# NREL/sup3r

Measured on AMD Instinct MI355X. Metric: samples/sec (lo-res chunks), generator forward, 5x/12x ST-GAN, higher is better.
Workload: dtype bf16

## Files before the change

### include/sup3r_hip.h

```cpp
#ifndef SUP3R_HIP_H
#define SUP3R_HIP_H

#include <stdint.h>

#ifdef __cplusplus
extern "C" {
#endif

#define S3_OK 0
#define S3_EINVAL (-1)
#define S3_EHIP (-2)
#define S3_ENOMEM (-3)
#define S3_ERCCL (-4)
#define S3_ESTATE (-5)
#define S3_ETIMEOUT (-6)

enum {
  S3_OP_CONV = 1,
  S3_OP_REPEAT_T = 2,
  S3_OP_D2S = 3,
  S3_OP_ACT = 4,
  S3_OP_ADD = 5,
  S3_OP_CONCAT = 6,
  S3_OP_DENSE = 7,
  S3_OP_PAD = 8,
  S3_OP_CROP = 9,
  S3_OP_VIEW = 10,
  S3_OP_ROLL_T = 11,
  S3_OP_DILATE = 12
};
enum { S3_ACT_NONE = 0, S3_ACT_RELU = 1, S3_ACT_LEAKY = 2 };
enum { S3_PAD_ZERO = 0, S3_PAD_REFLECT = 1 };
enum {
  S3_PREC_F32 = 0,
  S3_PREC_BF16 = 1,
  S3_PREC_BF16X3 = 2
};
enum { S3_LOSS_MAE = 0, S3_LOSS_MSE = 1, S3_LOSS_EXP = 2 };
enum { S3_BUF_W = 0, S3_BUF_G = 1, S3_BUF_M = 2, S3_BUF_V = 3 };

typedef struct s3_ctx s3_ctx;
typedef struct s3_params s3_params;
typedef struct s3_plan s3_plan;

typedef struct {
  int64_t dims[5];
} s3_tensor_desc;

typedef struct {
  int32_t kind;
  int32_t in0, in1, res, out;
  int32_t w, b;
  int32_t k[3], stride[3], lo[3], hi[3];
  int32_t pad_mode;
  int32_t act;
  float alpha;
  int32_t d2s;
  int32_t rep;
  int32_t bcast_c;
  int32_t reserved[4];
} s3_op_desc;

int s3_ctx_create(int device_id, void* stream, int create_stream, s3_ctx** out);
void s3_ctx_destroy(s3_ctx* ctx);
const char* s3_last_error(const s3_ctx* ctx);
int s3_ctx_sync(s3_ctx* ctx);
void* s3_ctx_stream(s3_ctx* ctx);
enum { S3_STAT_PERSIST_DGRAD = 0,
       S3_STAT_GCONV_SPLITK = 1,
       S3_STAT_BUCKET_ELEMS = 2,
       S3_STAT_DGRAD_C2_SLIDE = 3,
       S3_STAT_BUCKETS = 4,
       S3_STAT_ALLREDUCES = 5,
       S3_STAT_BIAS_STAGE1 = 6,
       S3_STAT_BIAS_STAGE1_V4 = 7,
       S3_STAT_BIAS_COLS = 8,
       S3_STAT_BIAS_COLS_SPLIT = 9,
       S3_STAT_BIAS_PARTIAL = 10,
       S3_STAT_BIAS_PARTIAL_RIDE = 11,
       S3_STAT_BIAS_PARTIAL_FLUSH = 12,
       S3_STAT_EPI_GENERIC = 13,
       S3_STAT_EPI_C4 = 14,
       S3_STAT_EPI_D2S4 = 15,
       S3_STAT_EPI_C4_BSUM = 16,
       S3_STAT_EPI_D2S4_BSUM = 17,
       S3_STAT_FOLD_GATHER = 18,
       S3_STAT_FOLD_PAD4 = 19,
       S3_STAT_FOLD_PAD4_FR16 = 20,
       S3_STAT_FOLD16X8 = 21,
       S3_STAT_FOLD_PLAIN = 22,
       S3_STAT_FOLD_MASKED = 23,
       S3_STAT_FOLD_ADD = 24,
       S3_STAT_AXPY = 25,
       S3_STAT_AXPY4 = 26,
       S3_STAT_PERSIST_SKIPPRE = 27,
       S3_STAT_HALO_S2_K64 = 28,
       S3_STAT_FEWCH_HALO = 29,
       S3_STAT_FEWCH_HALO_SIGNS = 30,
       S3_STAT_DGRAD_S2_O16 = 31,
       S3_STAT_DGRAD_S2_MB = 32,
       S3_STAT_COUNT = 33 };
int64_t s3_ctx_stat(const s3_ctx* ctx, int which);

int s3_params_create(s3_ctx* ctx, int n, const int64_t* sizes, s3_params** out);
void s3_params_destroy(s3_params* p);
int64_t s3_params_total(const s3_params* p);
int s3_params_set(s3_params* p, int which, int idx, const float* host);
int s3_params_get(s3_params* p, int which, int idx, float* host);
void* s3_params_dptr(s3_params* p, int which, int idx);
int s3_params_zero_grad(s3_params* p);
uint64_t s3_params_version(const s3_params* p);
int s3_params_mean_abs(s3_params* p, int which, int idx, float* host_out);

int s3_adam_step(s3_params* p, float lr, float beta1, float beta2, float eps,
                 int64_t t);
typedef enum {
  S3_OPT_ADAM = 0, S3_OPT_SGD = 1, S3_OPT_RMSPROP = 2, S3_OPT_ADAGRAD = 3,
  S3_OPT_ADAMAX = 4, S3_OPT_ADAMW = 5
} s3_optimizer_kind;
int s3_optimizer_step(s3_params* p, int kind, const double* hp, int n_hp,
                      int64_t t);
int s3_optimizer_stage(s3_params* p, int kind, const double* hp, int n_hp,
                       int64_t t);
int s3_optimizer_step_staged(s3_params* p, int kind);
int s3_params_touch(s3_params* p);

typedef struct s3_graph s3_graph;
int s3_capture_begin(s3_ctx* ctx);
int s3_capture_end(s3_ctx* ctx, s3_graph** out);
int s3_capture_abort(s3_ctx* ctx);
int s3_graph_launch(s3_graph* g);
int64_t s3_graph_nodes(const s3_graph* g);
void s3_graph_destroy(s3_graph* g);

#define S3_OPTION_UNSET INT32_MIN
typedef struct {
  int32_t n;
  const char* const* names;
  const int32_t* values;
} s3_plan_options;
int s3_ctx_set_option(s3_ctx* ctx, const char* name, int32_t value);
int s3_ctx_get_option(const s3_ctx* ctx, const char* name, int32_t* value);
const char* s3_option_name_at(int index);

int s3_plan_create(s3_ctx* ctx, s3_params* params, const s3_tensor_desc* tensors,
                   int n_tensors, const s3_op_desc* ops, int n_ops,
                   const int32_t* inputs, int n_inputs, int32_t output,
                   int precision, int training, s3_plan** out);
int s3_plan_create_opt(s3_ctx* ctx, s3_params* params, const s3_tensor_desc* tensors,
                       int n_tensors, const s3_op_desc* ops, int n_ops,
                       const int32_t* inputs, int n_inputs, int32_t output,
                       int precision, int training, const s3_plan_options* options,
                       s3_plan** out);
void s3_plan_destroy(s3_plan* plan);
int s3_plan_forward(s3_plan* plan, const void* const* inputs, void* output);
int s3_plan_supports_window(const s3_plan* plan);
int s3_plan_forward_window(s3_plan* plan, const void* const* inputs, void* output,
                           const int64_t* lo3, const int64_t* n3,
                           const float* affine_dev, int n_c);
int s3_plan_backward(s3_plan* plan, const void* d_output, void* d_input,
                     int need_wgrad, int accumulate_wgrad);
void* s3_plan_tensor(s3_plan* plan, int32_t tensor_id);
int64_t s3_plan_workspace_bytes(const s3_plan* plan);
int s3_plan_profile_begin(s3_plan* plan, int max_forwards);
int s3_plan_profile_end(s3_plan* plan, float* ms_per_op, int cap);
int s3_plan_op_is_mfma(const s3_plan* plan, int op_index);
enum {
  S3_OPINFO_KIND = 0,
  S3_OPINFO_FWD = 1,
  S3_OPINFO_IN16 = 2,
  S3_OPINFO_OUT16 = 3,
  S3_OPINFO_RES16 = 4,
  S3_OPINFO_FWD_BF16_OPS = 5,
  S3_OPINFO_WGRAD = 6,
  S3_OPINFO_DGRAD = 7,
  S3_OPINFO_MASK_FUSED_FROM = 8,
  S3_OPINFO_IN_REP = 9,
  S3_OPINFO_RES_REP = 10,
  S3_OPINFO_DGRAD_FRAME16 = 11,
  S3_OPINFO_FEWPOS_MFMA = 12,
  S3_OPINFO_COUNT = 13
};
enum {
  S3_FWD_DIRECT = 0, S3_FWD_MFMA_TILE = 1, S3_FWD_MFMA_PERSIST = 2, S3_FWD_GCONV = 3,
// ... 378 lines not shown
```

### sup3r_amd/_lib.py

```python
import ctypes as C
import os

HERE = os.path.dirname(os.path.abspath(__file__))
LIB_PATH = os.environ.get('SUP3R_AMD_LIB') or os.path.join(
    HERE, 'lib', 'libsup3r_hip.so')

PREC_F32, PREC_BF16, PREC_BF16X3 = 0, 1, 2
LOSS_MAE, LOSS_MSE, LOSS_EXP = 0, 1, 2
BUF_W, BUF_G, BUF_M, BUF_V = 0, 1, 2, 3
OPT_ADAM = 0
SURF_OTHER, SURF_TEMP, SURF_PRES, SURF_RH = 0, 1, 2, 3
E_TIMEOUT = -6
PRECISIONS = {'f32': PREC_F32, 'bf16': PREC_BF16, 'bf16x3': PREC_BF16X3}

EXPORTS = [
    's3_ctx_create', 's3_ctx_destroy', 's3_last_error', 's3_ctx_sync',
    's3_ctx_stream', 's3_ctx_stat', 's3_params_create', 's3_params_destroy',
    's3_params_total', 's3_params_set', 's3_params_get', 's3_params_dptr',
    's3_params_zero_grad', 's3_params_version', 's3_params_mean_abs',
    's3_adam_step', 's3_optimizer_step', 's3_optimizer_stage',
    's3_optimizer_step_staged', 's3_params_touch', 's3_capture_begin',
    's3_capture_end', 's3_capture_abort', 's3_graph_launch', 's3_graph_nodes',
    's3_graph_destroy',
    's3_ctx_set_option', 's3_ctx_get_option', 's3_option_name_at',
# ... 230 lines not shown
        's3_scale_to_time_max': (i32, [vp, vp, vp, i64, i64, vp]),
        's3_host_register': (i32, [vp, vp, C.c_size_t]),
        's3_host_unregister': (i32, [vp, vp]),
        's3_d2h_window': (i32, [vp, vp, vp, i64, i64, i64, i64, i64, vp]),
        's3_d2h_stream': (i32, [vp, vp, vp, C.c_size_t, vp, i32]),
        's3_host_alloc': (i32, [vp, C.c_size_t, i32, C.POINTER(vp)]),
        's3_host_free': (i32, [vp, vp]),
        's3_d2h_async': (i32, [vp, vp, vp, C.c_size_t, vp]),
        's3_dma_d2h_begin': (i32, [vp, vp, vp, C.c_size_t,
                                   C.POINTER(C.c_uint64)]),
        's3_dma_wait': (i32, [vp, C.c_uint64, i32]),
        's3_coarsen': (i32, [vp, vp, i32, i32, i32, i32, i32, i32, i32, i32,
                             vp]),
        's3_gaussian_smooth': (i32, [vp, vp, i32, i32, i32, i32, i32, pf, i32,
                                     C.c_uint32, vp, vp]),
        's3_condmom_target': (i32, [vp, vp, vp, vp, i32, i32, i32, i32, i32,
                                    i32, i32, C.POINTER(i32), i32, i32,
                                    C.c_uint32, i32, i32, i32, vp, vp]),
        's3_sample_gather': (i32, [vp, vp, i64, i64, i64, i32, C.POINTER(i32),
                                   i32, i32, i32, i32, C.POINTER(i32), i32,
                                   vp]),
        's3_cc_night_mask': (i32, [vp, vp, i64, i64, i64, i32, C.POINTER(i32),
                                   i32, i32, i32, i32, vp]),
        's3_cc_window_gather': (i32, [vp, vp, i64, i64, i64, i32,
                                      C.POINTER(i32), i32, i32, i32, i32,
                                      C.POINTER(i32), i32, vp, vp]),
        's3_nn_fill': (i32, [vp, vp, i32, i32, i32, i32, i32, i32, vp, vp]),
        's3_channel_moments': (i32, [vp, vp, i64, i32, vp]),
        's3_normalize_channels': (i32, [vp, vp, i64, i32, pf, pf,
                                        C.POINTER(C.c_ubyte)]),
        's3_bias_correct': (i32, [vp, vp, i32, i32, i32, i32, i32,
                                  C.POINTER(BiasChannel), i32, i32,
                                  C.POINTER(i32), vp, vp, vp,
                                  C.POINTER(C.c_double),
                                  C.POINTER(C.c_double), i32, vp, vp]),
        's3_bc_base_series': (i32, [vp, vp, vp, i64, i64, i32, vp, vp, vp, vp,
                                    i32, vp, vp, vp, vp, i32, C.c_uint32, i32,
                                    i64, i64, vp]),
        's3_bc_moments': (i32, [vp, vp, i32, i64, vp, vp, i32, vp, vp, vp]),
        's3_bc_window_quantiles': (i32, [vp, vp, i32, i64, i32, vp, vp, vp,
                                         vp, i32, vp]),
        's3_bc_match_zero_rate': (i32, [vp, vp, i64, vp, i32, i64, vp, vp]),
        's3_bc_presrat': (i32, [vp, vp, i64, vp, i64, vp, i64, i32, i32, i32,
                                vp, vp, vp, i32, C.c_double, vp, vp,
                                C.POINTER(vp), C.POINTER(vp), C.POINTER(vp),
                                C.POINTER(vp), vp, vp, vp, vp, vp, vp, vp]),
        's3_st_interp': (i32, [vp, vp, i32, i32, i32, i32, i32, i32, i32, vp,
                               vp]),
        's3_resize2d': (i32, [vp, vp, i32, i32, i32, i32, i32, vp, vp, vp, vp,
                              i32, vp, vp]),
        's3_surface_downscale': (i32, [vp, vp, i32, i32, i32, i32, i32, vp, vp,
                                       vp, vp, i32, vp, vp, vp, i32, vp, u64,
                                       C.c_uint32, vp, vp, vp, vp, vp, vp]),
        's3_comm_unique_id': (i32, [vp]),
        's3_comm_init': (i32, [vp, i32, i32, vp]),
        's3_params_allreduce_grads': (i32, [vp]),
        's3_params_arm_allreduce': (i32, [vp, i64]),
        's3_allreduce_sum': (i32, [vp, vp, i64]),
        's3_comm_info': (i32, [vp, C.POINTER(i32), C.POINTER(i32)]),
        's3_params_broadcast': (i32, [vp, i32, i32]),
        's3_broadcast': (i32, [vp, vp, i64, i32]),
        's3_comm_destroy': (None, [vp]),
        's3_comm_wait': (i32, [vp, i64]),
        's3_version': (C.c_char_p, []),
    }
    for name in EXPORTS:
        fn = getattr(L, name)
        fn.restype, fn.argtypes = sig[name]
    _lib = L
    return L


STATS = {'persist_dgrad': 0, 'gconv_splitk': 1, 'bucket_elems': 2,
         'dgrad_c2_slide': 3, 'buckets': 4, 'allreduces': 5,
         'bias_stage1': 6, 'bias_stage1_v4': 7, 'bias_cols': 8,
         'bias_cols_split': 9, 'bias_partial': 10, 'bias_partial_ride': 11,
         'bias_partial_flush': 12, 'epi_generic': 13, 'epi_c4': 14,
         'epi_d2s4': 15, 'epi_c4_bsum': 16, 'epi_d2s4_bsum': 17,
         'fold_gather': 18, 'fold_pad4': 19, 'fold_pad4_fr16': 20,
         'fold16x8': 21, 'fold_plain': 22, 'fold_masked': 23, 'fold_add': 24,
         'axpy': 25, 'axpy4': 26,
         'persist_skippre': 27,
         'halo_s2_k64': 28, 'fewch_halo': 29, 'fewch_halo_signs': 30,
         'dgrad_s2_o16': 31, 'dgrad_s2_mb': 32}


def option_names():
    L, out, i = lib(), [], 0
    while True:
        name = L.s3_option_name_at(i)
        if not name:
            return out
        out.append(name.decode())
        i += 1


def plan_options(options):
    items = sorted((options or {}).items())
    n = len(items)
    names = (C.c_char_p * max(n, 1))(*[k.encode() for k, _ in items])
    values = (C.c_int32 * max(n, 1))(*[
        OPTION_UNSET if v is None else int(v) for _, v in items])
    return PlanOptions(n, names, values), (names, values)

OPINFO_FIELDS = ('kind', 'fwd', 'in16', 'out16', 'res16', 'fwd_bf16_ops',
                 'wgrad', 'dgrad', 'mask_fused_from', 'in_rep', 'res_rep',
                 'dgrad_frame16', 'fewpos_mfma')
FWD_KERNELS = ('direct', 'mfma_tile', 'mfma_persist', 'gconv', 'gconv_fewch',
               'halo32', 'fewpos', 'tail_mfma', 'small', 'fused2d', 'halo_s2',
               'mfma_gen', 'conv2d_ws', 'conv2d_head')
WGRAD_KERNELS = ('direct', 'f32_trunk', 'bf16_trunk', 'f32_gen', 'bf16_gen',
                 'bf16_2d', 'c2', 'tail', 'fewpos')
DGRAD_KERNELS = ('direct', 'mfma_frame', 'mfma_valid', 'mfma_chunked',
                 'fewch_frame', 's2', 'c2', 'gconv', 'fewpos')

TC_METHODS = {'subsample': 0, 'average': 1, 'total': 2, 'max': 3, 'min': 4}
CM_SUBFILTER, CM_LINEAR, CM_MOM1, CM_SQUARE = 1, 2, 4, 8
SAMPLE_MAX_ORIGINS, SAMPLE_MAX_CHANNELS = 64, 32
STATS_MAX_CHANNELS = 64
CC_STATUS_WORDS = 4
CC_NIGHT_MASK, CC_START_RAW, CC_START, CC_FILLED = 0, 1, 2, 3
NN_FILL_MAX_AXIS = 2048
BC_MAX_CHANNELS, BC_MAX_CHUNKS = 16, 32
BC_NONE, BC_LINEAR, BC_QDM = 0, 1, 2
(BC_MONTH, BC_WEIGHTS, BC_SCALAR_RANGE, BC_ADDER_RANGE, BC_OUT_RANGE,
 BC_PER_CHUNK, BC_RELATIVE, BC_NO_TREND, BC_DENOM_ZERO, BC_DENOM_MIN,
 BC_DELTA_RANGE, BC_PRESRAT, BC_GLOBAL) = (1 << i for i in range(13))
BCC_MAX_SORT, BCC_MAX_GROUPS = 32768, 12
BCC_AVG, BCC_MAX, BCC_MIN, BCC_SUM, BCC_NONE = range(5)
BCC_NANSKIP, BCC_CS_RATIO, BCC_ROUND = 1, 2, 4
BCC_PR_BIAS_NONFINITE, BCC_PR_FUT_NONFINITE, BCC_PR_INDEX = 0, 1, 2
LI_MAX_LEVELS, LI_MAX_SINGLE, LI_MAX_VARS, LI_MAX_TARGETS = 64, 8, 8, 16
LI_LINEAR, LI_LOG = 0, 1
LI_LEV_COLUMN, LI_LEV_VECTOR = 0, 1
(DP_UV_FROM_WSWD, DP_WSWD_FROM_UV, DP_SURFACE_RH, DP_RATIO_MASKED,
 DP_CLOUD_MASK, DP_RATIO_CLIP01, DP_ADD, DP_SCALE, DP_OFFSET, DP_BCAST_PIXEL,
 DP_BCAST_TIME) = range(11)
TF_LE, TF_NAN = 0, 1
STACK_MAX_PLANES = 32
LS_WORDS = 8
(LS_NAN, LS_BAD_MIN, LS_BAD_MAX, LS_ALL_NAN, LS_FIRST_MAX, LS_FIRST_MIN,
 LS_LAST_MAX, LS_LAST_MIN) = range(8)
EXO_MAX_SLAB = 32
QA_CUBE, QA_TIME_FIRST = 0, 1
QA_MAX_FEATURES, QA_SUMMARY_WORDS, QA_MAX_BINS = 16, 5, 4096
QA_HIST_STATS, QA_HIST_COUNTS, QA_HIST_KEEP_ALL = 1, 2, 4
RG_GRID, RG_FLAT, RG_FLAT_1D = 0, 1, 2
DAILY_MAX_SRC, DAILY_MAX_OUT = 8, 16
DAILY_MEAN, DAILY_MAX, DAILY_MIN, DAILY_SUM, DAILY_RATIO = range(5)


def last_error(ctx):
    raw = lib().s3_last_error(ctx) if ctx else None
    return raw.decode() if raw else ''


def check(rc, ctx=None, what=''):
    if rc == 0:
        return
    msg = ''
    if ctx:
        raw = lib().s3_last_error(ctx)
        msg = raw.decode() if raw else ''
    if rc == E_TIMEOUT:
        raise TimeoutError(f'sup3r_amd: {msg or what}')
    raise RuntimeError(f'sup3r_amd HIP call failed ({what}, code {rc}): {msg}')
```

### sup3r_amd/csrc/common.h

```cpp
#pragma once
#include <hip/hip_runtime.h>
#include <stdint.h>

#include <atomic>
#include <mutex>
#include <string>
#include <vector>

#include "../../include/sup3r_hip.h"
#include "launch_shape.h"


#define S3_OPTION_LIST(X) \
  X(BF16_TRAIN_ACT) \
  X(DENSE_WGS) \
  X(DGRAD_S2_MIN_TILES) \
  X(DISC_BF16) \
  X(FEWCH_HALO_MIN_TILES) \
  X(FP32_ACT) \
  X(GCONV_MF2) \
  X(GCONV_MF4) \
  X(GRAPH) \
  X(HALO32_MIN_TILES) \
  X(HALO_S2_MIN_TILES) \
  X(MFMA_DBG) \
  X(MFMA_TILE) \
  X(NO_BATCHED_PACK) \
  X(NO_BIAS_FUSE) \
  X(NO_CHUNKED_DY16) \
  X(NO_DGRAD_C2) \
  X(NO_DGRAD_C2_SLIDE) \
  X(DGRAD_C2_SLIDE_MIN_UNITS) \
  X(NO_DGRAD_CHUNKED) \
  X(NO_DGRAD_FEWCH) \
  X(NO_DGRAD_S2) \
  X(NO_DGRAD_X3) \
  X(NO_DIRECT_OUTPUT) \
  X(NO_DISC_BF16) \
  X(NO_DPRE16) \
  X(NO_DPRE16_ONLY_MASK) \
  X(NO_FEWCH) \
  X(NO_FEWCH_HALO) \
  X(NO_FEWPOS) \
  X(NO_FEWPOS_MFMA) \
  X(NO_FEWPOS_BWD_FUSE) \
  X(NO_FEWPOS_SMALL) \
  X(NO_FEWPOS_TRUNK) \
  X(NO_FOLD16) \
  X(NO_FRAME16) \
  X(NO_FUSED2D) \
  X(NO_GCONV) \
  X(NO_GCONV_DY16) \
  X(NO_GCONV_SPLITK) \
  X(NO_HALO32) \
  X(NO_HALO_S2) \
  X(NO_MASK_FUSE) \
  X(NO_MFMA_GEN) \
  X(NO_DGRAD_GEN) \
  X(NO_CONV2D_WS) \
  X(NO_TRAIN2D_BF16) \
  X(NO_ADD16) \
  X(NO_WS_EXO) \
  X(NO_WS_RES2) \
  X(NO_WS_PP) \
  X(NO_WS_X3) \
  X(WS_X3_MIN_POS) \
  X(NO_CONV2D_OUT) \
  X(NO_CONV2D_HEAD) \
  X(KEEP_ACTIVATIONS) \
  X(NO_MFMA_BWD) \
  X(NO_PERSIST) \
  X(NO_PERSIST_DGRAD) \
  X(NO_PERSIST_SKIPPRE) \
  X(NO_PERSIST_STRIP) \
  X(PERSIST2) \
  X(NO_REPEAT_FUSE) \
  X(NO_WGRAD_X3) \
  X(NO_GCONV_X3) \
  X(NO_SIGN_BYTES) \
  X(NO_HALO_S2_K64) \
  X(NO_PLAIN_FOLD16) \
  X(NO_SEG_REDUCE) \
  X(NO_TAIL_BAND) \
  X(NO_TAIL_MFMA) \
  X(NO_TAIL_SLIDE) \
  X(NO_TAIL_SWEEP) \
  X(NO_TAIL_WINDOW) \
  X(NO_TAIL_X3) \
  X(NO_TILE66) \
  X(NO_TILE_NF2) \
  X(NO_WGRAD_BF16) \
  X(NO_WGRAD_C2) \
  X(NO_WGRAD_GEN_PF) \
  X(NO_WGRAD_TAIL) \
  X(NO_WGRAD_TAIL_SWEEP) \
  X(NO_WGRAD_WS) \
  X(PERSIST_DGRAD_MIN_TILES) \
  X(PERSIST_MIN_TILES) \
  X(POISON_ALLOC) \
  X(TAIL_SWEEP_SHAPE) \
  X(TRACE) \
  X(WGRAD_DBG) \
  X(WGRAD_SIDE_STREAM)
enum S3OptId {
#define X(n) S3O_##n,
  S3_OPTION_LIST(X)
#undef X
  S3O_COUNT
};
struct S3Options {
  int32_t v[S3O_COUNT];
  bool has[S3O_COUNT];
  S3Options() { for (int i = 0; i < S3O_COUNT; ++i) { v[i] = 0; has[i] = false; } }
};
extern thread_local const S3Options* s3_active_options;
const char* s3_option_name(int id);
int s3_option_id(const char* name);
inline bool s3_opt_has(int id) { return s3_active_options && s3_active_options->has[id]; }
inline long long s3_opt_int(int id, long long dflt) { return s3_opt_has(id) ? s3_active_options->v[id] : dflt; }
inline bool s3_opt_on(int id) { return s3_opt_int(id, 0) != 0; }
struct S3OptScope {
  const S3Options* prev;
  explicit S3OptScope(const S3Options* o) : prev(s3_active_options) { s3_active_options = o; }
  ~S3OptScope() { s3_active_options = prev; }
};

struct s3_ctx {
  int device = 0;
  hipStream_t stream = nullptr;
  bool own_stream = false;
  std::string err;
  void* comm = nullptr;
  int rank = 0, nranks = 1;
  float* scratch = nullptr;
  size_t scratch_bytes = 0;
  int num_cu = 256;
  size_t lds_max = 64 * 1024;
  int64_t stat[S3_STAT_COUNT] = {};
  S3Options opt;
  hipStream_t comm_stream = nullptr;
  hipEvent_t comm_ev[2] = {nullptr, nullptr};
  hipEvent_t wd_ev[2] = {nullptr, nullptr};
  int64_t comm_issued = 0;
  hipStream_t wg_stream = nullptr;
  hipEvent_t wg_ev[2] = {nullptr, nullptr};
  bool wg_forked = false;
  hipStream_t cap_stream = nullptr, saved_stream = nullptr;
  bool capturing = false;
  bool graphs_made = false;
  std::vector<void*> retired;
  struct PendingBias { const float* partial = nullptr; int nblk = 0, c = 0; float* db = nullptr; int accumulate = 0; } pend_bias;
};

struct S3DeviceOnce {
  std::atomic<uint64_t> mask{0};
// ... 404 lines not shown
```

### sup3r_amd/csrc/kernels_conv_mfma_persist.hip

```cpp
#include <cstdlib>

#include "wave_prims.h"

namespace {

constexpr int TS0 = 4, TS1 = 8, TS2 = 16;
constexpr int H0 = TS0 + 2, H1 = TS1 + 2, H2 = TS2 + 2;
constexpr int HP = H0 * H1 * H2;
constexpr int HALO_BYTES = HP * 128;
constexpr int SLAB_OFF = HALO_BYTES;
constexpr int BIAS_OFF = SLAB_OFF + 3 * 8192;
constexpr int LDS_BYTES = BIAS_OFF + 256;

constexpr int NCW = 8;
constexpr int NPW = 4;
constexpr int NTHR = (NCW + NPW) * 64;
constexpr int MFW = TS0 * TS1 / NCW;
constexpr int PT = NPW * 64;
constexpr int ROWC = H1 * H2;
constexpr int JR = (ROWC * 8 + PT - 1) / PT;
constexpr int NLATE = (H0 - 2) * JR;
static_assert(MFW * NCW == TS0 * TS1 && TS1 % MFW == 0 && MFW == 4, "tile / wave split");
static_assert(JR <= 6 && NLATE <= 24, "producer tap schedule");

// ... 437 lines not shown
#pragma unroll
        for (int h = 0; h < 2; ++h) {
          if (2 * h >= NFV) continue;
          f32x4 a0 = acc[m][(2 * h) % NFV], a1 = acc[m][(2 * h + 1) % NFV];
          if constexpr (F16) {
            uint4 o;
            o.x = pk2(a0[0], a0[1]); o.y = pk2(a0[2], a0[3]);
            o.z = pk2(a1[0], a1[1]); o.w = pk2(a1[2], a1[3]);
            *reinterpret_cast<uint4*>(y + yo + h * 32) = o;
            continue;
          }
          if (res) {
            const float4 p0 = *reinterpret_cast<const float4*>(yp + h * 32);
            const float4 p1 = *reinterpret_cast<const float4*>(yp + h * 32 + 4);
            a0[0] += p0.x; a0[1] += p0.y; a0[2] += p0.z; a0[3] += p0.w;
            a1[0] += p1.x; a1[1] += p1.y; a1[2] += p1.z; a1[3] += p1.w;
          }
          *reinterpret_cast<float4*>(yp + h * 32) = make_float4(a0[0], a0[1], a0[2], a0[3]);
          *reinterpret_cast<float4*>(yp + h * 32 + 4) = make_float4(a1[0], a1[1], a1[2], a1[3]);
        }
      }
      WG_BARRIER();
      continue;
    }
    const size_t e_base = (size_t)n * g.O[0] * g.O[1] * g.O[2] * g.Cout;
    if constexpr (!SKP) {
      EPI_POS()
    }
#undef EPI_POS
    auto chunk_off = [&](int m, int h, bool& ok) __attribute__((always_inline)) {
      ok = c_ok[h] && e_ok[m] && 2 * h < NFV;
      return e_pos[m] + c_off[h];
    };
    if (!SKP && res) {
      const bool rr = REP > 1 && !DG && g.res_rep > 1;
      const int O2s = rr ? g.O[2] / (REP > 1 ? REP : 1) : g.O[2];
      const size_t r_base = rr ? (size_t)n * g.O[0] * g.O[1] * O2s * g.Cout : e_base;
#pragma unroll
      for (int m = 0; m < MFW; ++m) {
        unsigned r_pos = e_pos[m];
        if (rr) {
          const int mf = mf0 + m;
          const int o0 = org0 + mf / TS1, o1 = org1 + mf % TS1, o2 = org2 + frow;
          r_pos = (unsigned)(((o0 * g.O[1] + o1) * O2s + o2 / (REP > 1 ? REP : 1)) * cpo);
        }
#pragma unroll
        for (int h = 0; h < 2; ++h) {
          bool ok;
          chunk_off(m, h, ok);
          rres[m][h] = make_uint4(0, 0, 0, 0);
          if (ok) rres[m][h] = *reinterpret_cast<const uint4*>(res + r_base + r_pos + c_off[h]);
        }
      }
    }
#pragma unroll
    for (int m = 0; m < MFW; ++m) {
#pragma unroll
      for (int h = 0; h < 2; ++h) {
        bool ok;
        const unsigned off = chunk_off(m, h, ok);
        if (!ok) continue;
        float v[8];
#pragma unroll
        for (int q = 0; q < 8; ++q) {
          const float a = acc[m][(2 * h + (q >> 2)) % NFV][q & 3];
          const float sa = slope * a;
          asm("v_max_f32 %0, %1, %2" : "=v"(v[q]) : "v"(a), "v"(sa));
        }
        if (SKP || res) {
          const uint4 r = rres[m][h];
          v[0] += bf_lo(r.x); v[1] += bf_hi(r.x); v[2] += bf_lo(r.y); v[3] += bf_hi(r.y);
          v[4] += bf_lo(r.z); v[5] += bf_hi(r.z); v[6] += bf_lo(r.w); v[7] += bf_hi(r.w);
        }
        uint4 o;
        o.x = pk2(v[0], v[1]); o.y = pk2(v[2], v[3]);
        o.z = pk2(v[4], v[5]); o.w = pk2(v[6], v[7]);
        *reinterpret_cast<uint4*>(y + e_base + off) = o;
      }
    }
    WG_BARRIER();
  }
}

}

bool conv_mfma_persist_geom_ok(const ConvGeom& g) {
  if (g.Cin != 64 || g.Cout % 8 != 0 || g.Cout < 64 || g.d2s < 1) return false;
  if (g.D[2] < 8) return false;
  if (g.d2s > 1 && (g.Cout % (g.d2s * g.d2s) != 0 || (g.Cout / (g.d2s * g.d2s)) % 8 != 0))
    return false;
  if (g.pad_mode != S3_PAD_REFLECT) return false;
  if (g.act == S3_ACT_LEAKY && !(g.alpha >= 0.f && g.alpha <= 1.f)) return false;
  for (int d = 0; d < 3; ++d)
    if (g.k[d] != 3 || g.s[d] != 1) return false;
  return (int64_t)g.D[0] * g.D[1] * g.D[2] * 64 < (int64_t)1 << 31 &&
         (int64_t)g.O[0] * g.O[1] * g.O[2] * g.Cout < (int64_t)1 << 31;
}

bool conv_mfma_persist_dgrad_geom_ok(const ConvGeom& g) {
  if (g.Cin != 64 || (g.Cout != 64 && g.Cout != 32) || g.d2s != 1 || g.pad_mode != S3_PAD_ZERO ||
      g.act != S3_ACT_NONE)
    return false;
  for (int d = 0; d < 3; ++d)
    if (g.k[d] != 3 || g.s[d] != 1 || g.lo[d] != 2 || g.O[d] != g.D[d] + 2) return false;
  if (g.D[2] < 8) return false;
  if (g.in_cstride && ((g.in_cstride & 7) || (g.in_cvalid & 7) || g.in_cvalid < 8 || g.in_cvalid > 64)) return false;
  return (int64_t)g.N * g.D[0] * g.D[1] * g.D[2] * (g.in_cstride ? g.in_cstride : 64) < (int64_t)1 << 28;
}

static void persist_dgrad_grid(const ConvGeom& g, int* gs0, int* gs1) {
  int64_t best = -1;
  for (int a = 1; a <= g.N; ++a) {
    if (g.N % a) continue;
    const int b = g.N / a;
    const int64_t t = (int64_t)((a * g.O[0] + 1) / 2) * ((b * g.O[1] + TS1 - 1) / TS1);
    if (best < 0 || t < best) { best = t; *gs0 = a; *gs1 = b; }
  }
}

bool conv_mfma_persist_dgrad_supported(const s3_ctx* ctx, const ConvGeom& g) {
  if (s3_opt_on(S3O_NO_PERSIST_DGRAD)) return false;
  if (!conv_mfma_persist_dgrad_geom_ok(g)) return false;
  int gs0 = 1, gs1 = 1;
  persist_dgrad_grid(g, &gs0, &gs1);
  const int64_t halves = (int64_t)((gs0 * g.O[0] + 1) / 2) * ((gs1 * g.O[1] + TS1 - 1) / TS1) *
                         ((g.O[2] + TS2 - 1) / TS2);
  const int64_t tiles = (int64_t)((gs0 * g.O[0] + TS0 - 1) / TS0) * ((gs1 * g.O[1] + TS1 - 1) / TS1) *
                        ((g.O[2] + TS2 - 1) / TS2);
  const int64_t covered = halves * 2 * TS1 * TS2;
  const int64_t six = (int64_t)g.N * ((g.O[0] + 5) / 6) * ((g.O[1] + 5) / 6) * ((g.O[2] + 15) / 16) * 576;
  const int64_t min_tiles = s3_opt_has(S3O_PERSIST_DGRAD_MIN_TILES)
                                ? s3_opt_int(S3O_PERSIST_DGRAD_MIN_TILES, 0) : ctx->num_cu;
  return tiles >= min_tiles && covered * 10 <= six * 11;
}

int launch_conv_mfma_persist_dgrad(s3_ctx* ctx, const ConvGeom& g, const void* dpre16, const void* image,
                                   float* dxp, int accumulate, int frame16) {
  static S3DeviceOnce attr_set;
  if (int rc = s3_lds_optin(ctx, attr_set,
                            conv3_mfma_persist_kernel<4, true>, LDS_BYTES,
                            conv3_mfma_persist_kernel<2, true>, LDS_BYTES,
                            conv3_mfma_persist_kernel<4, true, 0, false, true>, LDS_BYTES)) return rc;
  if (frame16 && (accumulate || g.Cout != 64))
    S3_FAIL(ctx, S3_ESTATE, "persistent data gradient: a bf16 frame is written once, 64 channels wide");
  int gs0 = 1, gs1 = 1;
  persist_dgrad_grid(g, &gs0, &gs1);
  const int tiles0 = (gs0 * g.O[0] + 1) / 2, tiles1 = (gs1 * g.O[1] + TS1 - 1) / TS1,
            tiles2 = (g.O[2] + TS2 - 1) / TS2;
  const int n_tiles = tiles0 * tiles1 * tiles2;
  const int grid = persistent_grid(ctx->num_cu, (n_tiles + 1) / 2);
  auto kern = g.Cout <= 32 ? conv3_mfma_persist_kernel<2, true> : conv3_mfma_persist_kernel<4, true>;
  if (frame16) kern = conv3_mfma_persist_kernel<4, true, 0, false, true>;
  hipLaunchKernelGGL(kern, dim3(grid), dim3(NTHR), LDS_BYTES, ctx->stream,
                     (const unsigned short*)dpre16, (const char*)image, (const float*)nullptr,
                     (const unsigned short*)(accumulate ? dxp : nullptr), (unsigned short*)dxp, g, tiles0, tiles1,
                     tiles2, n_tiles, 0, gs0, gs1);
  S3_HIP(ctx, hipGetLastError());
  ++ctx->stat[S3_STAT_PERSIST_DGRAD];
  return S3_OK;
}

bool conv_mfma_persist_rep_ok(int rep) { return rep == 2 || rep == 3 || rep == 4; }

bool conv_mfma_persist_supported(const s3_ctx* ctx, const ConvGeom& g, ConvIO io,
                                 bool has_res) {
  if (s3_opt_on(S3O_NO_PERSIST)) return false;
  if (!io.in_bf16 || !io.out_bf16 || (has_res && !io.res_bf16)) return false;
  if (!conv_mfma_persist_geom_ok(g)) return false;
  if (has_res && g.d2s != 1) return false;
  const int64_t tiles = (int64_t)g.N * ((g.O[0] + TS0 - 1) / TS0) *
                        ((g.O[1] + TS1 - 1) / TS1) * ((g.O[2] + TS2 - 1) / TS2);
  return tiles >= s3_opt_int(S3O_PERSIST_MIN_TILES, ctx->num_cu * 7 / 16);
}

int launch_pack_jobs(s3_ctx* ctx, const S3PackJob* jobs_dev, int n_jobs, int max_ct) {
  if (n_jobs <= 0) return S3_OK;
  hipLaunchKernelGGL(pack_jobs_kernel, dim3(108 * max_ct, n_jobs), dim3(256), 0, ctx->stream, jobs_dev);
  S3_HIP(ctx, hipGetLastError());
  return S3_OK;
}

size_t conv_mfma_persist_image_bytes(const ConvGeom& g) {
  return (size_t)((g.Cout + 63) / 64) * 27 * 64 * 64 * 2;
}

int launch_conv_mfma_persist_pack(s3_ctx* ctx, const ConvGeom& g, const float* w, void* image) {
  const int n_ct = (g.Cout + 63) / 64;
  hipLaunchKernelGGL(pack_persist_kernel, dim3(108 * n_ct), dim3(256), 0, ctx->stream,
                     w, (unsigned short*)image, g.Cout, n_ct);
  S3_HIP(ctx, hipGetLastError());
  return S3_OK;
}

int launch_conv_mfma_persist(s3_ctx* ctx, const ConvGeom& g, const void* x,
                             const void* image, const float* bias,
                             const void* res, void* y) {
  static S3DeviceOnce attr_set;
#define S3_REP_ATTR(R)                                                                \
  conv3_mfma_persist_kernel<4, false, R, true>, LDS_BYTES,                            \
  conv3_mfma_persist_kernel<4, false, R, false>, LDS_BYTES,                           \
  conv3_mfma_persist_kernel<4, false, R, true, false, 6>, PGeo<6>::LDS_BYTES,         \
  conv3_mfma_persist_kernel<4, false, R, false, false, 6>, PGeo<6>::LDS_BYTES
  if (int rc = s3_lds_optin(ctx, attr_set,
                            conv3_mfma_persist_kernel<4, false>, LDS_BYTES,
                            conv3_mfma_persist_kernel<2, false>, LDS_BYTES,
                            conv3_mfma_persist_kernel<4, false, 0, false, false, 8, true>, LDS_BYTES,
                            S3_REP_ATTR(2), S3_REP_ATTR(3), S3_REP_ATTR(4),
                            conv3_mfma_persist_kernel<4, false, 0, false, false, 6>, PGeo<6>::LDS_BYTES,
                            conv3_mfma_persist_kernel<2, false, 0, false, false, 6>, PGeo<6>::LDS_BYTES)) return rc;
#undef S3_REP_ATTR
  const int tiles0 = (g.O[0] + 1) / 2, tiles1 = (g.O[1] + TS1 - 1) / TS1,
            tiles2 = (g.O[2] + TS2 - 1) / TS2;
  const int n_tiles = g.N * tiles0 * tiles1 * tiles2;
  const int grid = persistent_grid(ctx->num_cu, (n_tiles + 1) / 2);
  const int n_ct = (g.Cout + 63) / 64;
  const int rep = g.in_rep > 1 ? g.in_rep : (g.res_rep > 1 ? g.res_rep : 0);
  const bool rin = g.in_rep > 1;
  const bool skp = res && !rep && g.d2s == 1 && g.Cout == 64 && !s3_opt_on(S3O_NO_PERSIST_SKIPPRE);
  if (skp) ++ctx->stat[S3_STAT_PERSIST_SKIPPRE];
  ConvGeom gk = g;
  if (rep) {
    bool ok = conv_mfma_persist_rep_ok(rep) && g.Cout == 64 && g.d2s == 1 &&
              !(g.in_rep > 1 && g.res_rep > 1 && g.in_rep != g.res_rep);
    for (int d = 0; d < 3; ++d) ok = ok && g.lo[d] == g.lo[0] && g.O[d] == g.D[d];
    if (!ok) S3_FAIL(ctx, S3_ESTATE, "persistent conv: unsupported fused temporal repeat");
    if (rin) gk.D[2] = g.D[2] / rep;
  }
  const int rem1 = g.O[1] % TS1;
  const int64_t strip_halves = (int64_t)g.N * tiles0 * tiles2;
  if (rem1 >= 1 && rem1 <= 6 && g.O[1] > TS1 && strip_halves >= 2 * (int64_t)ctx->num_cu &&
      (!rep || n_ct == 1) && !s3_opt_on(S3O_NO_PERSIST_STRIP)) {
    const int t1a = g.O[1] / TS1;
    const int na = g.N * tiles0 * t1a * tiles2, nb = (int)strip_halves;
    const int ga = persistent_grid(ctx->num_cu, (na + 1) / 2), gb = persistent_grid(ctx->num_cu, (nb + 1) / 2);
    for (int ct = 0; ct < n_ct; ++ct) {
      const bool half = g.Cout - ct * 64 <= 32;
      const char* img = (const char*)image + (size_t)ct * 27 * 8192;
      auto k8 = half ? conv3_mfma_persist_kernel<2, false> : conv3_mfma_persist_kernel<4, false>;
      auto k6 = half ? conv3_mfma_persist_kernel<2, false, 0, false, false, 6>
                     : conv3_mfma_persist_kernel<4, false, 0, false, false, 6>;
      if (skp) k8 = conv3_mfma_persist_kernel<4, false, 0, false, false, 8, true>;
      if (rep == 2) {
        k8 = rin ? conv3_mfma_persist_kernel<4, false, 2, true> : conv3_mfma_persist_kernel<4, false, 2, false>;
        k6 = rin ? conv3_mfma_persist_kernel<4, false, 2, true, false, 6>
                 : conv3_mfma_persist_kernel<4, false, 2, false, false, 6>;
      } else if (rep == 3) {
        k8 = rin ? conv3_mfma_persist_kernel<4, false, 3, true> : conv3_mfma_persist_kernel<4, false, 3, false>;
        k6 = rin ? conv3_mfma_persist_kernel<4, false, 3, true, false, 6>
                 : conv3_mfma_persist_kernel<4, false, 3, false, false, 6>;
      } else if (rep == 4) {
        k8 = rin ? conv3_mfma_persist_kernel<4, false, 4, true> : conv3_mfma_persist_kernel<4, false, 4, false>;
        k6 = rin ? conv3_mfma_persist_kernel<4, false, 4, true, false, 6>
                 : conv3_mfma_persist_kernel<4, false, 4, false, false, 6>;
      }
      hipLaunchKernelGGL(k8, dim3(ga), dim3(NTHR), LDS_BYTES, ctx->stream, (const unsigned short*)x, img, bias,
                         (const unsigned short*)res, (unsigned short*)y, gk, tiles0, t1a, tiles2, na, ct, 1, 0);
      hipLaunchKernelGGL(k6, dim3(gb), dim3(NTHR), PGeo<6>::LDS_BYTES, ctx->stream, (const unsigned short*)x,
                         img, bias, (const unsigned short*)res, (unsigned short*)y, gk, tiles0, 1, tiles2, nb,
                         ct, 1, t1a * TS1);
    }
    S3_HIP(ctx, hipGetLastError());
    return S3_OK;
  }
  for (int ct = 0; ct < n_ct; ++ct) {
    const bool half = g.Cout - ct * 64 <= 32;
    auto kern = half ? conv3_mfma_persist_kernel<2, false> : conv3_mfma_persist_kernel<4, false>;
    if (skp) kern = conv3_mfma_persist_kernel<4, false, 0, false, false, 8, true>;
    if (rep == 2) kern = rin ? conv3_mfma_persist_kernel<4, false, 2, true> : conv3_mfma_persist_kernel<4, false, 2, false>;
    else if (rep == 3) kern = rin ? conv3_mfma_persist_kernel<4, false, 3, true> : conv3_mfma_persist_kernel<4, false, 3, false>;
    else if (rep == 4) kern = rin ? conv3_mfma_persist_kernel<4, false, 4, true> : conv3_mfma_persist_kernel<4, false, 4, false>;
    hipLaunchKernelGGL(kern, dim3(grid), dim3(NTHR), LDS_BYTES, ctx->stream,
                       (const unsigned short*)x, (const char*)image + (size_t)ct * 27 * 8192, bias,
                       (const unsigned short*)res, (unsigned short*)y, gk, tiles0,
                       tiles1, tiles2, n_tiles, ct, 1, 0);
  }
  S3_HIP(ctx, hipGetLastError());
  return S3_OK;
}
```

Before: 2078.

## Fuse all output-channel passes of persistent conv into one kernel per tile

Adds a multi-pass persistent conv kernel that, for layers with 2-4 output-channel tiles and no residual or repeat, loads each input halo into LDS once and loops over all 64-channel weight passes before moving to the next tile. This replaces one launch per channel tile, each of which re-read the same input halos from global memory. In exchange, each tile now serialises more taps and barriers, and the producer waves must stream weight slabs for every pass. The path is on by default and can be turned off with a new NO_PERSIST_MULTITILE option, which also adds a stat counter.

Result: no change. 2079 (median of 6 runs) (+0.1%).

```diff
diff --git a/include/sup3r_hip.h b/include/sup3r_hip.h
--- a/include/sup3r_hip.h
+++ b/include/sup3r_hip.h
@@ -99,7 +99,8 @@
        S3_STAT_FEWCH_HALO_SIGNS = 30,
        S3_STAT_DGRAD_S2_O16 = 31,
        S3_STAT_DGRAD_S2_MB = 32,
-       S3_STAT_COUNT = 33 };
+       S3_STAT_PERSIST_MULTITILE = 33,
+       S3_STAT_COUNT = 34 };
 int64_t s3_ctx_stat(const s3_ctx* ctx, int which);
 
 int s3_params_create(s3_ctx* ctx, int n, const int64_t* sizes, s3_params** out);
diff --git a/sup3r_amd/_lib.py b/sup3r_amd/_lib.py
--- a/sup3r_amd/_lib.py
+++ b/sup3r_amd/_lib.py
@@ -336,7 +336,8 @@
          'axpy': 25, 'axpy4': 26,
          'persist_skippre': 27,
          'halo_s2_k64': 28, 'fewch_halo': 29, 'fewch_halo_signs': 30,
-         'dgrad_s2_o16': 31, 'dgrad_s2_mb': 32}
+         'dgrad_s2_o16': 31, 'dgrad_s2_mb': 32,
+         'persist_multitile': 33}
 
 
 def option_names():
diff --git a/sup3r_amd/csrc/common.h b/sup3r_amd/csrc/common.h
--- a/sup3r_amd/csrc/common.h
+++ b/sup3r_amd/csrc/common.h
@@ -71,6 +71,7 @@
   X(NO_MFMA_BWD) \
   X(NO_PERSIST) \
   X(NO_PERSIST_DGRAD) \
+  X(NO_PERSIST_MULTITILE) \
   X(NO_PERSIST_SKIPPRE) \
   X(NO_PERSIST_STRIP) \
   X(PERSIST2) \
diff --git a/sup3r_amd/csrc/kernels_conv_mfma_persist.hip b/sup3r_amd/csrc/kernels_conv_mfma_persist.hip
--- a/sup3r_amd/csrc/kernels_conv_mfma_persist.hip
+++ b/sup3r_amd/csrc/kernels_conv_mfma_persist.hip
@@ -543,6 +543,293 @@
   }
 }
 
+constexpr int MT_MAX_CT = 4;
+constexpr int MT_LDS_BYTES = BIAS_OFF + MT_MAX_CT * 256;
+static_assert(MT_LDS_BYTES <= 160 * 1024, "bias block of the multi-tile form");
+
+template <int NCT, int NFL>
+__global__ __launch_bounds__(NTHR) void conv3_mfma_persist_multi_kernel(
+    const unsigned short* __restrict__ x, const char* __restrict__ wimg,
+    const float* __restrict__ bias, unsigned short* __restrict__ y, ConvGeom g,
+    int tiles0, int tiles1, int tiles2, int n_tiles) {
+  static_assert(NCT >= 2 && NCT <= MT_MAX_CT && (NFL == 2 || NFL == 4), "channel passes");
+  extern __shared__ __attribute__((aligned(16))) char smem[];
+  const int tid = threadIdx.x;
+  const int lane = tid & 63;
+  const int wave = __builtin_amdgcn_readfirstlane(tid >> 6);
+  const int D0 = g.D[0], D1 = g.D[1], D2 = g.D[2];
+
+  int h_cur, h_end;
+  {
+    const int nblk = gridDim.x, b = blockIdx.x;
+    const int xcd = b % 8, k = b / 8;
+    int rank = k;
+    for (int xx = 0; xx < xcd; ++xx) rank += (nblk - xx + 7) / 8;
+    const long long H = n_tiles;
+    h_cur = (int)((rank * H) / nblk);
+    h_end = (int)(((rank + 1) * H) / nblk);
+  }
+  auto tile_org = [&](int h, int& n, int& o0, int& o1, int& o2) __attribute__((always_inline)) {
+    int tr = h;
+    o0 = (tr % tiles0) * 2; tr /= tiles0;
+    o2 = (tr % tiles2) * TS2; tr /= tiles2;
+    o1 = (tr % tiles1) * TS1; tr /= tiles1;
+    n = tr;
+  };
+  auto item_at = [&](int h, int& hs0, int& nr) __attribute__((always_inline)) {
+    const bool whole = hs0 + 1 < tiles0 && h + 1 < h_end;
+    nr = whole ? 4 : 2;
+    hs0 += whole ? 2 : 1;
+    if (hs0 >= tiles0) hs0 = 0;
+    return h + (whole ? 2 : 1);
+  };
+
+  if (wave >= NCW) {
+    const int pt = tid - NCW * 64;
+    const int pw = wave - NCW;
+    const unsigned dma_voff = (unsigned)(pw * 2048 + lane * 16);
+    auto dma_slab = [&](int s, int slot) __attribute__((always_inline)) {
+      unsigned vo;
+      asm volatile("v_mov_b32 %0, %1" : "=v"(vo) : "v"(dma_voff));
+      const char* sb = wimg + (vo + (unsigned)s * 8192u);
+      char* d = smem + SLAB_OFF + slot * 8192 + __builtin_amdgcn_readfirstlane((int)vo);
+      __builtin_amdgcn_global_load_lds(
+          (const __attribute__((address_space(1))) void*)sb,
+          (__attribute__((address_space(3))) void*)d, 16, 0, 0);
+      __builtin_amdgcn_global_load_lds(
+          (const __attribute__((address_space(1))) void*)(sb + 1024),
+          (__attribute__((address_space(3))) void*)(d + 1024), 16, 0, 0);
+    };
+    const int pcell = pt >> 3, pch = pt & 7;
+    u32x4 hlate[NLATE], hrow[JR];
+    unsigned in_off[JR];
+    unsigned lds_off[JR];
+    int htab = 0;
+    const unsigned short* hx = x;
+#pragma unroll
+    for (int j = 0; j < JR; ++j) {
+      int cell = pcell + 32 * j;
+      if (cell > ROWC - 1) cell = ROWC - 1;
+      lds_off[j] = (unsigned)(cell * 128 + ((pch ^ ((cell % H2) & 7)) << 4));
+    }
+#define MT_HALO_TABLE(tile_expr)                                                       \
+    {                                                                                  \
+      int n_, o0_, o1_, o2_;                                                           \
+      tile_org((tile_expr), n_, o0_, o1_, o2_);                                        \
+      n_ = __builtin_amdgcn_readfirstlane(n_);                                         \
+      const int ax = lane < H0 ? 0 : (lane < H0 + H1 ? 1 : 2);                         \
+      const int c = lane - (ax == 0 ? 0 : (ax == 1 ? H0 : H0 + H1));                   \
+      const int org = ax == 0 ? o0_ : (ax == 1 ? o1_ : o2_);                           \
+      const int D = ax == 0 ? D0 : (ax == 1 ? D1 : D2);                                \
+      const int stride = ax == 0 ? D1 * D2 * 64 : (ax == 1 ? D2 * 64 : 64);            \
+      int i = s3_reflect(org + c - g.lo[ax], D);                                       \
+            \
+      i = i < 0 ? 0 : (i > D - 1 ? D - 1 : i);                                         \
+      htab = i * stride;                                                               \
+      hx = x + (size_t)n_ * D0 * D1 * D2 * 64;                                         \
+      _Pragma("unroll") for (int j = 0; j < JR; ++j) {                                 \
+        int cell = pcell + 32 * j;                                                     \
+        if (cell > ROWC - 1) cell = ROWC - 1;                                          \
+        const int c1 = cell / H2, c2 = cell - c1 * H2;                                 \
+        in_off[j] = (unsigned)__builtin_amdgcn_ds_bpermute((H0 + c1) << 2, htab) +     \
+                    (unsigned)__builtin_amdgcn_ds_bpermute((H0 + H1 + c2) << 2, htab) + \
+                    pch * 8;                                                           \
+      }                                                                                \
+    }
+    auto halo_load = [&](int r, int j) __attribute__((always_inline)) {
+      const unsigned row = (unsigned)__builtin_amdgcn_readlane(htab, r);
+      return ld16_async(hx, (row + in_off[j]) * 2);
+    };
+    auto halo_put = [&](int r, int j, const u32x4& v) __attribute__((always_inline)) {
+      if (pcell + 32 * j < ROWC)
+        *reinterpret_cast<u32x4*>(smem + r * (ROWC * 128) + lds_off[j]) = v;
+    };
+
+    if (pt < 64 * NCT) {
+      const int co = (pt >> 6) * 64 + slab_row_cout(pt & 63);
+      reinterpret_cast<float*>(smem + BIAS_OFF)[pt] = (bias && co < g.Cout) ? bias[co] : 0.f;
+    }
+    dma_slab(0, 0);
+    dma_slab(1, 1);
+    if (h_cur < h_end) {
+      MT_HALO_TABLE(h_cur);
+#pragma unroll
+      for (int r = 0; r < H0; ++r) {
+#pragma unroll
+        for (int j = 0; j < JR; ++j) hrow[j] = halo_load(r, j);
+        WAIT_VM(0);
+#pragma unroll
+        for (int j = 0; j < JR; ++j) halo_put(r, j, hrow[j]);
+      }
+    }
+    WAIT_VM(0);
+    WAIT_LGKM0();
+    WG_BARRIER();
+
+    for (int h = h_cur; h < h_end;) {
+      int nr_, hs0_ = h % tiles0;
+      h = item_at(h, hs0_, nr_);
+#define has_next (h < h_end)
+#pragma unroll
+      for (int p = 0; p + 1 < NCT; ++p) {
+#pragma unroll
+        for (int tap = 0; tap < 27; ++tap) {
+          dma_slab(p * 27 + tap + 2, (tap + 2) % 3);
+          WAIT_VM(2);
+          WG_BARRIER();
+        }
+        WG_BARRIER();
+      }
+      MT_HALO_TABLE(h < h_end - 1 ? h : h_end - 1);
+#pragma unroll
+      for (int tap = 0; tap < 27; ++tap) {
+        if ((tap == 9 || tap == 18) && has_next) {
+#pragma unroll
+          for (int j = 0; j < JR; ++j) halo_put(tap == 9 ? 0 : 1, j, hrow[j]);
+        }
+        dma_slab(((NCT - 1) * 27 + tap + 2) % (27 * NCT), (tap + 2) % 3);
+        if (tap < JR) hrow[tap % JR] = halo_load(0, tap % JR);
+        if (tap >= 9 && tap < 9 + JR) hrow[(tap - 9) % JR] = halo_load(1, (tap - 9) % JR);
+        if (tap < NLATE) hlate[tap % NLATE] = halo_load(2 + (tap % NLATE) / JR, (tap % NLATE) % JR);
+        wait_vm_n(2 + halo_k(tap) + halo_k(tap - 1));
+        WG_BARRIER();
+      }
+      if (has_next) {
+#pragma unroll
+        for (int u = 0; u < NLATE; ++u) halo_put(2 + u / JR, u % JR, hlate[u]);
+      }
+      WAIT_LGKM0();
+      WG_BARRIER();
+#undef has_next
+    }
+#undef MT_HALO_TABLE
+    return;
+  }
+
+  const int frow = lane & 15, kq = lane >> 4;
+  const int mf0 = wave * MFW;
+  const int row0 = (mf0 / TS1) * H1 + (mf0 % TS1);
+  unsigned a_addr[3][2], b_addr[2];
+#pragma unroll
+  for (int c = 0; c < 3; ++c) {
+    const int sw = (frow + c) & 7;
+#pragma unroll
+    for (int ks = 0; ks < 2; ++ks)
+      a_addr[c][ks] = (unsigned)((row0 * H2 + frow + c) * 128 + (((ks * 4 + kq) ^ sw) << 4));
+  }
+#pragma unroll
+  for (int ks = 0; ks < 2; ++ks)
+    b_addr[ks] = (unsigned)(SLAB_OFF + frow * 128 + (((ks * 4 + kq) ^ ((frow >> 1) & 7)) << 4));
+  const float slope = g.act == S3_ACT_LEAKY ? g.alpha : (g.act == S3_ACT_RELU ? 0.f : 1.f);
+  const int db = g.d2s, cpo = g.Cout / (db * db);
+  unsigned c_off[2];
+  bool c_ok[2];
+#define MT_CHUNKS(p)                                                                               \
+  _Pragma("unroll") for (int hh = 0; hh < 2; ++hh) {                                               \
+    const int co = (p) * 64 + hh * 32 + kq * 8;                                                    \
+    c_ok[hh] = co < g.Cout;                                                                        \
+    const int blk = co / cpo;                                                                      \
+    c_off[hh] = (unsigned)((((blk / db) * (g.O[1] * db) + blk % db) * g.O[2]) * cpo + co % cpo);   \
+  }
+  MT_CHUNKS(0)
+  WG_BARRIER();
+  __builtin_amdgcn_s_setprio(2);
+
+  const int my_row = mf0 / TS1;
+  for (int h = h_cur; h < h_end;) {
+    int nr, n, org0, org1, org2;
+    tile_org(h, n, org0, org1, org2);
+    {
+      int hs0 = org0 >> 1;
+      h = item_at(h, hs0, nr);
+    }
+    if (my_row >= nr) {
+#pragma unroll 1
+      for (int t = 0; t < 28 * NCT; ++t) WG_BARRIER();
+      continue;
+    }
+    const size_t e_base = (size_t)n * g.O[0] * g.O[1] * g.O[2] * g.Cout;
+#define MT_TAP(NF, ta_off, tb, tc, NEXT_A)                                                         \
+    {                                                                                              \
+      bf16x8 bfr[NF];                                                                              \
+      _Pragma("unroll") for (int nf = 0; nf < NF; ++nf)                                            \
+        bfr[nf] = *reinterpret_cast<const bf16x8*>(smem + b_addr[0] + nf * 2048 + (tc) * 8192);    \
+      _Pragma("unroll") for (int m = 0; m < MFW; ++m)                                              \
+        _Pragma("unroll") for (int nf = 0; nf < NF; ++nf)                                          \
+          acc[m][nf] = __builtin_amdgcn_mfma_f32_16x16x32_bf16(bfr[nf], apre[m], acc[m][nf], 0, 0, 0); \
+      _Pragma("unroll") for (int nf = 0; nf < NF; ++nf)                                            \
+        bfr[nf] = *reinterpret_cast<const bf16x8*>(smem + b_addr[1] + nf * 2048 + (tc) * 8192);    \
+      _Pragma("unroll") for (int m = 0; m < MFW; ++m) {                                            \
+        const bf16x8 afr = *reinterpret_cast<const bf16x8*>(                                       \
+            smem + a_addr[tc][1] + (ta_off) + ((m + (tb)) * H2) * 128);                            \
+        _Pragma("unroll") for (int nf = 0; nf < NF; ++nf)                                          \
+          acc[m][nf] = __builtin_amdgcn_mfma_f32_16x16x32_bf16(bfr[nf], afr, acc[m][nf], 0, 0, 0); \
+      }                                                                                            \
+      {                                                                                            \
+        const int ntc = (tc) < 2 ? (tc) + 1 : 0;                                                   \
+        const int ntb = (tc) < 2 ? (tb) : ((tb) < 2 ? (tb) + 1 : 0);                               \
+        const unsigned nta_off = ((tc) == 2 && (tb) == 2) ? (ta_off) + H1 * H2 * 128 : (ta_off);   \
+        if (NEXT_A) {                                                                              \
+          _Pragma("unroll") for (int m = 0; m < MFW; ++m)                                          \
+            apre[m] = *reinterpret_cast<const bf16x8*>(                                            \
+                smem + a_addr[ntc][0] + nta_off + ((m + ntb) * H2) * 128);                         \
+        }                                                                                          \
+      }                                                                                            \
+      WG_BARRIER();                                                                                \
+    }
+#define MT_PASS(NF)                                                                                \
+    {                                                                                              \
+      f32x4 acc[MFW][NF];                                                                          \
+      _Pragma("unroll") for (int nf = 0; nf < NF; ++nf) {                                          \
+        const f32x4 bv = *reinterpret_cast<const f32x4*>(                                          \
+            smem + BIAS_OFF + p * 256 + (nf * 16 + kq * 4) * 4);                                   \
+        _Pragma("unroll") for (int m = 0; m < MFW; ++m) acc[m][nf] = bv;                           \
+      }                                                                                            \
+      bf16x8 apre[MFW];                                                                            \
+      _Pragma("unroll") for (int m = 0; m < MFW; ++m)                                              \
+        apre[m] = *reinterpret_cast<const bf16x8*>(smem + a_addr[0][0] + (m * H2) * 128);          \
+      _Pragma("unroll 1") for (int ta = 0; ta < 3; ++ta) {                                         \
+        const unsigned ta_off = (unsigned)(ta * H1 * H2 * 128);                                    \
+        _Pragma("unroll") for (int tb = 0; tb < 3; ++tb) {                                         \
+          _Pragma("unroll") for (int tc = 0; tc < 3; ++tc)                                         \
+            MT_TAP(NF, ta_off, tb, tc, (!(tc == 2 && tb == 2) || ta < 2))                          \
+        }                                                                                          \
+      }                                                                                            \
+      _Pragma("unroll") for (int m = 0; m < MFW; ++m) {                                            \
+        const int mf = mf0 + m;                                                                    \
+        const int o0 = org0 + mf / TS1, o1 = org1 + mf % TS1, o2 = org2 + frow;                    \
+        const bool e_ok = o0 < g.O[0] && o1 < g.O[1] && o2 < g.O[2];                               \
+        const unsigned e_pos = (unsigned)(((o0 * db * (g.O[1] * db) + o1 * db) * g.O[2] + o2) * cpo); \
+        _Pragma("unroll") for (int hh = 0; 2 * hh < NF; ++hh) {                                    \
+          if (!(c_ok[hh] && e_ok)) continue;                                                       \
+          float v[8];                                                                              \
+          _Pragma("unroll") for (int q = 0; q < 8; ++q) {                                          \
+                         \
+            const float a = acc[m][2 * hh + (q >> 2)][q & 3];                                      \
+            const float sa = slope * a;                                                            \
+            asm("v_max_f32 %0, %1, %2" : "=v"(v[q]) : "v"(a), "v"(sa));                            \
+          }                                                                                        \
+          uint4 o;                                                                                 \
+          o.x = pk2(v[0], v[1]); o.y = pk2(v[2], v[3]);                                            \
+          o.z = pk2(v[4], v[5]); o.w = pk2(v[6], v[7]);                                            \
+          *reinterpret_cast<uint4*>(y + e_base + (e_pos + c_off[hh])) = o;                         \
+        }                                                                                          \
+      }                                                                                            \
+      const int pn = p + 1 < NCT ? p + 1 : 0;                                                      \
+      MT_CHUNKS(pn)                                                                                \
+      WG_BARRIER();                                     \
+    }
+#pragma unroll 1
+    for (int p = 0; p < NCT; ++p) {
+      if (NFL == 2 && p == NCT - 1) MT_PASS(2)
+      else MT_PASS(4)
+    }
+#undef MT_PASS
+#undef MT_TAP
+  }
+#undef MT_CHUNKS
+}
+
 }
 
 bool conv_mfma_persist_geom_ok(const ConvGeom& g) {
@@ -668,7 +955,13 @@
                             conv3_mfma_persist_kernel<4, false, 0, false, false, 8, true>, LDS_BYTES,
                             S3_REP_ATTR(2), S3_REP_ATTR(3), S3_REP_ATTR(4),
                             conv3_mfma_persist_kernel<4, false, 0, false, false, 6>, PGeo<6>::LDS_BYTES,
-                            conv3_mfma_persist_kernel<2, false, 0, false, false, 6>, PGeo<6>::LDS_BYTES)) return rc;
+                            conv3_mfma_persist_kernel<2, false, 0, false, false, 6>, PGeo<6>::LDS_BYTES,
+                            conv3_mfma_persist_multi_kernel<2, 4>, MT_LDS_BYTES,
+                            conv3_mfma_persist_multi_kernel<2, 2>, MT_LDS_BYTES,
+                            conv3_mfma_persist_multi_kernel<3, 4>, MT_LDS_BYTES,
+                            conv3_mfma_persist_multi_kernel<3, 2>, MT_LDS_BYTES,
+                            conv3_mfma_persist_multi_kernel<4, 4>, MT_LDS_BYTES,
+                            conv3_mfma_persist_multi_kernel<4, 2>, MT_LDS_BYTES)) return rc;
 #undef S3_REP_ATTR
   const int tiles0 = (g.O[0] + 1) / 2, tiles1 = (g.O[1] + TS1 - 1) / TS1,
             tiles2 = (g.O[2] + TS2 - 1) / TS2;
@@ -723,6 +1016,17 @@
     S3_HIP(ctx, hipGetLastError());
     return S3_OK;
   }
+  if (n_ct >= 2 && n_ct <= MT_MAX_CT && !res && !rep && !s3_opt_on(S3O_NO_PERSIST_MULTITILE)) {
+    const bool half = g.Cout - (n_ct - 1) * 64 <= 32;
+    auto kern = half ? conv3_mfma_persist_multi_kernel<2, 2> : conv3_mfma_persist_multi_kernel<2, 4>;
+    if (n_ct == 3) kern = half ? conv3_mfma_persist_multi_kernel<3, 2> : conv3_mfma_persist_multi_kernel<3, 4>;
+    if (n_ct == 4) kern = half ? conv3_mfma_persist_multi_kernel<4, 2> : conv3_mfma_persist_multi_kernel<4, 4>;
+    hipLaunchKernelGGL(kern, dim3(grid), dim3(NTHR), MT_LDS_BYTES, ctx->stream, (const unsigned short*)x,
+                       (const char*)image, bias, (unsigned short*)y, gk, tiles0, tiles1, tiles2, n_tiles);
+    S3_HIP(ctx, hipGetLastError());
+    ++ctx->stat[S3_STAT_PERSIST_MULTITILE];
+    return S3_OK;
+  }
   for (int ct = 0; ct < n_ct; ++ct) {
     const bool half = g.Cout - ct * 64 <= 32;
     auto kern = half ? conv3_mfma_persist_kernel<2, false> : conv3_mfma_persist_kernel<4, false>;
```
